# vitasoftAI/ImageRetrievalResearch

Measured on AMD Instinct MI355X. Metric: images/sec embed + queries/sec top-k@100k-gallery, EffNet-B3a 224^2, higher is better.
Workload: dtype bf16

## Files before the change

imageretrievalresearch_amd/csrc/gemm_bf16.hip:

```cpp
#include "ops.h"
#include "../../include/mi355_retrieval.h"

#include <stdlib.h>

namespace mi355 {

typedef __bf16 bf16x8 __attribute__((ext_vector_type(8)));
typedef float f32x4 __attribute__((ext_vector_type(4)));
typedef unsigned u32x4 __attribute__((ext_vector_type(4)));
typedef unsigned u32x2 __attribute__((ext_vector_type(2)));

__device__ __forceinline__ float lo_bf(unsigned u) { return __uint_as_float(u << 16); }
__device__ __forceinline__ float hi_bf(unsigned u) { return __uint_as_float(u & 0xffff0000u); }

__device__ __forceinline__ u32x4 gate_chunk(u32x4 v, const float* __restrict__ gp, int relu6) {
    const f32x4 g0 = *reinterpret_cast<const f32x4*>(gp);
    const f32x4 g1 = *reinterpret_cast<const f32x4*>(gp + 4);
    float f[8] = {lo_bf(v.x) * g0.x, hi_bf(v.x) * g0.y, lo_bf(v.y) * g0.z, hi_bf(v.y) * g0.w,
                  lo_bf(v.z) * g1.x, hi_bf(v.z) * g1.y, lo_bf(v.w) * g1.z, hi_bf(v.w) * g1.w};
    if (relu6) {
#pragma unroll
        for (int i = 0; i < 8; ++i) f[i] = fminf(fmaxf(f[i], 0.f), 6.f);
    }
    u32x4 o;
    o.x = pack2bf(f[0], f[1]); o.y = pack2bf(f[2], f[3]); o.z = pack2bf(f[4], f[5]); o.w = pack2bf(f[6], f[7]);
    return o;
}

__device__ __forceinline__ u32x4 gate_chunk_regs(u32x4 v, f32x4 g0, f32x4 g1, int relu6) {
    float f[8] = {lo_bf(v.x) * g0.x, hi_bf(v.x) * g0.y, lo_bf(v.y) * g0.z, hi_bf(v.y) * g0.w,
                  lo_bf(v.z) * g1.x, hi_bf(v.z) * g1.y, lo_bf(v.w) * g1.z, hi_bf(v.w) * g1.w};
    if (relu6) {
#pragma unroll
// ... 617 lines not shown
}

template <int NT, int KST>
__global__ __launch_bounds__(512) void k_proj_lds(const GemmArgs g) {
    constexpr int NW = 8;
    constexpr int KP = KST * 32;
    constexpr int WLD = KP + 8, ALD = KP + 8, CLD = NT * 16 + 8;
    extern __shared__ __attribute__((aligned(16))) unsigned char psm[];
    bf16_t* Wsh = reinterpret_cast<bf16_t*>(psm);
    float* sbias = reinterpret_cast<float*>(psm + (size_t)NT * 16 * WLD * 2);
    unsigned char* wbase = psm + (size_t)NT * 16 * WLD * 2 + NT * 16 * 4;
    constexpr int WS = 16 * ALD * 2 + 16 * CLD * 2 + KP * 4;
    const int tid = threadIdx.x, lane = tid & 63;
    const int wave = __builtin_amdgcn_readfirstlane(tid >> 6);
    bf16_t* As = reinterpret_cast<bf16_t*>(wbase + (size_t)wave * WS);
    bf16_t* Cs = As + 16 * ALD;
    float* Gs = reinterpret_cast<float*>(Cs + 16 * CLD);
    const int Npad = (g.N + 15) & ~15;
    for (int id = tid; id < NT * 16 * KST * 4; id += 512) {
        const int row = id / (KST * 4), c = id - row * (KST * 4);
        u32x4 v = {0u, 0u, 0u, 0u};
        if (row < Npad && c * 8 < g.ldw) v = *reinterpret_cast<const u32x4*>(g.W + (size_t)row * g.ldw + c * 8);
        *reinterpret_cast<u32x4*>(&Wsh[row * WLD + c * 8]) = v;
    }
    for (int n = tid; n < NT * 16; n += 512) sbias[n] = n < Npad ? g.bias[n] : 0.f;
    for (int id = lane; id < 16 * (ALD / 8); id += 64) *reinterpret_cast<u32x4*>(&As[id * 8]) = (u32x4){0u, 0u, 0u, 0u};
    __syncthreads();

    const int fr = lane & 15, fq = lane >> 4;
    const int kc = g.K >> 3;
    const int nchunk = 16 * kc;
    const int ntiles = (g.M + 15) >> 4;
    const int stride = gridDim.x * NW;
    int img = -1;
    u32x4 sv[KST];
    auto stage_load = [&](int tile) {
#pragma unroll
        for (int i = 0; i < KST; ++i) {
            const int id = min(lane + 64 * i, nchunk - 1);
            const int row = id / kc, c = id - row * kc;
            const int m = min(tile * 16 + row, g.M - 1);
            sv[i] = *reinterpret_cast<const u32x4*>(g.A + (size_t)m * g.lda + c * 8);
        }
        __builtin_amdgcn_sched_barrier(0);
    };
    int tile = blockIdx.x * NW + wave;
    if (tile < ntiles) stage_load(tile);
    for (; tile < ntiles; tile += stride) {
        if (g.gate) {
            const int im = (tile * 16) / g.rows_per_img;
            if (im != img) {
                img = im;
                for (int k4 = lane; k4 * 4 < g.K; k4 += 64)
                    *reinterpret_cast<f32x4*>(&Gs[k4 * 4]) = *reinterpret_cast<const f32x4*>(g.gate + (size_t)im * g.gate_ld + k4 * 4);
            }
        }
#pragma unroll
        for (int i = 0; i < KST; ++i) {
            const int id = lane + 64 * i;
            if (id < nchunk) {
                const int row = id / kc, c = id - row * kc;
                u32x4 v = sv[i];
                if (g.gate) v = gate_chunk(v, Gs + c * 8, g.a_relu6);
                else if (g.a_relu6) v = relu6_chunk(v);
                *reinterpret_cast<u32x4*>(&As[row * ALD + c * 8]) = v;
            }
        }
        if (tile + stride < ntiles) stage_load(tile + stride);
        f32x4 acc[NT];
#pragma unroll
        for (int ni = 0; ni < NT; ++ni) acc[ni] = (f32x4){0.f, 0.f, 0.f, 0.f};
#pragma unroll
        for (int ks = 0; ks < KST; ++ks) {
            const bf16x8 af = *reinterpret_cast<const bf16x8*>(&As[fr * ALD + ks * 32 + fq * 8]);
#pragma unroll
            for (int ni = 0; ni < NT; ++ni) {
                const bf16x8 wf = *reinterpret_cast<const bf16x8*>(&Wsh[(ni * 16 + fr) * WLD + ks * 32 + fq * 8]);
                acc[ni] = __builtin_amdgcn_mfma_f32_16x16x32_bf16(wf, af, acc[ni], 0, 0, 0);
            }
        }
        MI355_ACT_DISPATCH(g.act, {
_Pragma("unroll")
            for (int ni = 0; ni < NT; ++ni) {
                const f32x4 bb = *reinterpret_cast<const f32x4*>(&sbias[ni * 16 + fq * 4]);
                acc[ni].x = act_c<ACT>(acc[ni].x + bb.x); acc[ni].y = act_c<ACT>(acc[ni].y + bb.y);
                acc[ni].z = act_c<ACT>(acc[ni].z + bb.z); acc[ni].w = act_c<ACT>(acc[ni].w + bb.w);
            }
        })
        const int m = tile * 16 + fr;
#pragma unroll
        for (int ni = 0; ni < NT; ++ni) {
            const int n = ni * 16 + fq * 4;
            float v[4] = {acc[ni].x, acc[ni].y, acc[ni].z, acc[ni].w};
            if (g.res && m < g.M && n < g.N) {
                if (n + 3 < g.res_n) {
                    const u32x2 rr = *reinterpret_cast<const u32x2*>(g.res + (size_t)m * g.ldr + n);
                    v[0] += lo_bf(rr.x); v[1] += hi_bf(rr.x); v[2] += lo_bf(rr.y); v[3] += hi_bf(rr.y);
                } else {
#pragma unroll
                    for (int r = 0; r < 4; ++r)
                        if (n + r < g.res_n) v[r] += bf2f(g.res[(size_t)m * g.ldr + n + r]);
                }
            }
            u32x2 o;
            o.x = pack2bf(v[0], v[1]);
            o.y = pack2bf(v[2], v[3]);
            *reinterpret_cast<u32x2*>(&Cs[fr * CLD + n]) = o;
        }
        constexpr int CPR = NT * 2;
#pragma unroll
        for (int i = 0; i < (16 * CPR + 63) / 64; ++i) {
            const int id = lane + 64 * i;
            const int row = id / CPR, c = id - row * CPR;
            const int mm = tile * 16 + row;
            if (id < 16 * CPR && mm < g.M && c * 8 < g.N)
                *reinterpret_cast<u32x4*>((bf16_t*)g.out + (size_t)mm * g.ldo + c * 8) =
                    *reinterpret_cast<const u32x4*>(&Cs[row * CLD + c * 8]);
        }
    }
}

template <int NT, int KST>
static int launch_proj_cfg(const GemmArgs& a, hipStream_t st) {
    constexpr int KP = KST * 32;
    const size_t lds = (size_t)NT * 16 * (KP + 8) * 2 + (size_t)NT * 16 * 4 +
                       (size_t)8 * (16 * (KP + 8) * 2 + 16 * (NT * 16 + 8) * 2 + KP * 4);
    static bool attr_done[MI355_MAX_DEVICES] = {false};
    if (first_time_on_this_device(attr_done)) {
        MI355_CHECK_HIP(hipFuncSetAttribute((const void*)k_proj_lds<NT, KST>, hipFuncAttributeMaxDynamicSharedMemorySize,
                                            160 * 1024));
    }
    const int ntiles = cdiv(a.M, 16);
    int blocks = cdiv(ntiles, 8);
    if (blocks > 256 * 6) blocks = 256 * 6;
    hipLaunchKernelGGL((k_proj_lds<NT, KST>), dim3(blocks), dim3(512), lds, st, a);
    MI355_LAUNCH_CHECK();
    return OK;
}

static int try_launch_proj(const GemmArgs& a, hipStream_t st, int* nt_out) {
    if (a.out_f32 || a.M < (1 << 19) || a.N % 8 || a.ldo % 8 || a.N > 64 || a.K > 288 || a.lda != a.K) return -1;
    if (a.gate && (a.rows_per_img % 16 != 0 || a.gate_ld % 4 != 0)) return -1;
    const int kst = (a.K + 31) / 32, nt = (a.N + 15) / 16;
#define PROJ_CASE(NTV, KSTV) if (nt == NTV && kst == KSTV) { *nt_out = NTV; return launch_proj_cfg<NTV, KSTV>(a, st); }
    PROJ_CASE(2, 1); PROJ_CASE(2, 2); PROJ_CASE(2, 5); PROJ_CASE(2, 6); PROJ_CASE(3, 6); PROJ_CASE(3, 9); PROJ_CASE(2, 9);
    PROJ_CASE(4, 8); PROJ_CASE(3, 5);
#undef PROJ_CASE
    return -1;
}

static int try_launch_stream(const GemmArgs& a, hipStream_t st, int* nt_out) {
    if (a.out_f32 || a.M < 4096 || a.N % 8 || a.ldo % 8 || a.gate || a.a_relu6) return -1;
    const int kst = (a.K + 31) / 32;
    const int nt = (a.N + 15) / 16;
    *nt_out = nt;
    if (kst == 1 && nt == 9) return launch_stream_cfg<9, 1>(a, st);
    if (kst == 1 && nt == 12) return launch_stream_cfg<12, 1>(a, st);
    return -1;
}

constexpr int SK_KC = 256, SK_BM = 64, SK_BN = 64, SK_LD = SK_KC + 8;
constexpr size_t SK_MAX_BYTES = (size_t)64 << 20;

int gemm_splitk_chunks(long M, int rows_per_img, int N, int K) {
    if (M > 16384 || rows_per_img > 196 || K < 512 || N < 64 || N % 8 || gemm_splitk_bytes(M, N, K) > SK_MAX_BYTES) return 0;
    return (K + SK_KC - 1) / SK_KC;
}
size_t gemm_splitk_bytes(long M, int N, int K) {
    return (size_t)((K + SK_KC - 1) / SK_KC) * (size_t)M * (size_t)((N + 15) & ~15) * sizeof(float);
}

__global__ __launch_bounds__(256) void k_gemm_splitk(const GemmArgs g, float* __restrict__ ws) {
    extern __shared__ __attribute__((aligned(16))) bf16_t sksm[];
    bf16_t* As = sksm;
    bf16_t* Ws = sksm + SK_BM * SK_LD;
// ... 348 lines not shown
```

imageretrievalresearch_amd/csrc/sweep_mbconv.hip:

```cpp
#include "../../include/mi355_retrieval.h"
#include "ops.h"

namespace mi355 {

typedef __bf16 bf16x8 __attribute__((ext_vector_type(8)));
typedef float f32x4 __attribute__((ext_vector_type(4)));
typedef unsigned u32x4 __attribute__((ext_vector_type(4)));
typedef unsigned u32x2 __attribute__((ext_vector_type(2)));

__device__ __forceinline__ void sw_lds_barrier() {
    asm volatile("s_waitcnt lgkmcnt(0)" ::: "memory");
    __builtin_amdgcn_s_barrier();
    asm volatile("" ::: "memory");
}

typedef __bf16 sw_bf16x2 __attribute__((ext_vector_type(2)));
typedef float sw_f32x2 __attribute__((ext_vector_type(2)));
__device__ __forceinline__ u32x2 sw_pack4(const f32x4 v) {
    const sw_bf16x2 lo = __builtin_convertvector((sw_f32x2){v.x, v.y}, sw_bf16x2);
    const sw_bf16x2 hi = __builtin_convertvector((sw_f32x2){v.z, v.w}, sw_bf16x2);
    u32x2 o;
    o.x = *reinterpret_cast<const unsigned*>(&lo);
    o.y = *reinterpret_cast<const unsigned*>(&hi);
    return o;
}

template <int ACT>
__device__ __forceinline__ float sw_act(float x, int act_runtime) {
    if constexpr (ACT >= 0) return act_c<ACT>(x);
    else return apply_act(x, act_runtime);
}

template <int KS> struct SwTaps {
    static constexpr int NV = (KS / 2) * KS;
    static constexpr int NH = (KS + 1) / 2;
    static constexpr int NP = NV + NH;
    __host__ __device__ static constexpr bool vertical(int tp) { return tp < NV; }
    __host__ __device__ static constexpr int tap_a(int tp) {
        return tp < NV ? (tp / KS) * 2 * KS + tp % KS : (KS - 1) * KS + (tp - NV) * 2;
    }
    __host__ __device__ static constexpr int tap_b(int tp) {
        return tp < NV ? tap_a(tp) + KS : ((tp - NV) * 2 + 1 < KS ? tap_a(tp) + 1 : -1);
    }
};

template <int KS, int S, int WI, int TH>
struct SwGeom {
    static constexpr int PAD = KS / 2;
    static constexpr int HALO = KS - S;
    static constexpr int NEWR = TH * S;
    static constexpr int IH = NEWR + HALO;
    static constexpr int EW = WI + 2 * PAD;
    static constexpr int EWH = (EW + 1) / 2;
    static constexpr int RP = S == 1 ? EW : 2 * EWH;
    static constexpr int HOFF = S == 1 ? 1 : EWH;
    static constexpr int WO = (WI + 2 * PAD - KS) / S + 1;
    static constexpr int ELD = 24;
    static constexpr int EBUF = (IH + 1) * RP * ELD;
    static constexpr size_t lds_bytes(int nw, int ns = 1) { return (size_t)ns * 2 * EBUF * 2 + (size_t)nw * 16 * ns * 4; }
    __host__ __device__ static constexpr int epx(int r, int c) {
        return r * RP + (S == 1 ? c : (c & 1) * EWH + (c >> 1));
    }
};

template <int KS, int S, int WI, int TH, int NW, int KST, int OCC, bool PREF, int AE, int AD, int NS = 1>
__global__ __launch_bounds__(NW * 64, (NW * OCC + 3) / 4) void k_sweep_mbconv(const SweepArgs a) {
    using G = SwGeom<KS, S, WI, TH>;
    using TP = SwTaps<KS>;
    constexpr int NTHR = NW * 64;
    constexpr int PAD = G::PAD, HALO = G::HALO, NEWR = G::NEWR, RP = G::RP, ELD = G::ELD, WO = G::WO, NP = TP::NP;
    constexpr int NPX1 = NEWR * WI, NT1 = (NPX1 + 15) / 16, MW1 = (NT1 + NW - 1) / NW;
    constexpr int NPX2 = TH * WO, NT2 = (NPX2 + 15) / 16, MW2 = (NT2 + NW - 1) / NW;
    constexpr int EBUF = G::EBUF;
    extern __shared__ __attribute__((aligned(16))) unsigned char sw_smem[];
    bf16_t* Es = reinterpret_cast<bf16_t*>(sw_smem);
    float* red = reinterpret_cast<float*>(sw_smem + (size_t)NS * 2 * EBUF * 2);

    const int tid = threadIdx.x, lane = tid & 63;
    const int wave = __builtin_amdgcn_readfirstlane(tid >> 6);
    const int fr = lane & 15, fq = lane >> 4, fk = fq * 8;
    const int xcd = blockIdx.x & 7, seq = blockIdx.x >> 3;
    const int b = xcd + 8 * (seq / a.csplit), g = seq % a.csplit;
    if (b >= a.B) return;
    const int midp = (a.mid + 15) & ~15;
    const int nslab = (midp / 16 + NS - 1) / NS;
    const int nbands = (a.Ho + TH - 1) / TH;

    const bool stamping = a.stamps != nullptr;
    long long t_acc[10] = {0, 0, 0, 0, 0, 0, 0, 0, 0, 0};
    long long t_last = 0;
    if (stamping) t_last = (long long)__builtin_readcyclecounter();
    auto tick = [&](int i) {
        if (stamping) { const long long t = (long long)__builtin_readcyclecounter(); t_acc[i] += t - t_last; t_last = t; }
    };

    for (int id = tid; id < NS * 2 * EBUF / 8; id += NTHR) *reinterpret_cast<u32x4*>(&Es[id * 8]) = (u32x4){0u, 0u, 0u, 0u};

    int eoff[MW1];
#pragma unroll
    for (int i = 0; i < MW1; ++i) {
        const int p = min((wave + NW * i) * 16 + fr, NPX1 - 1);
        const int r = p / WI, x = p - r * WI;
        eoff[i] = G::epx(HALO + r, x + PAD) * ELD + fq * 4;
    }
    int rbase[MW2];
#pragma unroll
    for (int i = 0; i < MW2; ++i) {
        const int p = min((wave + NW * i) * 16 + fr, NPX2 - 1);
        const int oyl = p / WO, ox = p - oyl * WO;
        rbase[i] = (oyl * S * RP + ox) * ELD + (fq & 1) * 8;
    }
    const int vsel = (fq >> 1) ? RP * ELD : 0;
    const int hsel = (fq >> 1) ? G::HOFF * ELD : 0;
    sw_lds_barrier();
    tick(0);

    const bf16_t* xb = a.X + (size_t)b * a.H * WI * a.Cin;
    bf16_t* Db = a.D + (size_t)b * a.Ho * WO * a.mid;
    const int hw1 = a.H * WI - 1;
    const int kclamp = a.Cin - 8;

    u32x4 xa[MW1][KST];
    auto load_x = [&](int band) {
        const int pix0 = (band * NEWR - PAD + HALO) * WI;
#pragma unroll
        for (int i = 0; i < MW1; ++i) {
            const int pix = min(max(pix0 + (wave + NW * i) * 16 + fr, 0), hw1);
#pragma unroll
            for (int ks = 0; ks < KST; ++ks) {
                u32x4 t = {0u, 0u, 0u, 0u};
                if (!(a.debug_skip & 4)) t = *reinterpret_cast<const u32x4*>(xb + pix * a.Cin + min(ks * 32 + fk, kclamp));
                xa[i][ks] = t;
            }
        }
        __builtin_amdgcn_sched_barrier(0);
    };

    for (int si = g; si < nslab; si += a.csplit) {
        const int ch0 = ((si + b) % nslab) * (16 * NS);
        load_x(-1);
        if constexpr (HALO > NEWR) {
            constexpr int NZ16 = (HALO - NEWR) * RP * ELD / 8;
#pragma unroll
            for (int s = 0; s < NS; ++s)
                for (int id = tid; id < NZ16; id += NTHR)
                    *reinterpret_cast<u32x4*>(&Es[s * 2 * EBUF + NEWR * RP * ELD + id * 8]) = (u32x4){0u, 0u, 0u, 0u};
        }
        u32x4 wf[NS][KST];
        f32x4 bb[NS], bdr[NS];
        unsigned wd_raw[NS][(NP + 1) / 2];
#pragma unroll
        for (int s = 0; s < NS; ++s) {
            const int c0 = ch0 + 16 * s;
            const int n = min(c0 + fr, midp - 1);
#pragma unroll
            for (int ks = 0; ks < KST; ++ks) wf[s][ks] = *reinterpret_cast<const u32x4*>(a.We + (n * a.Kp + ks * 32 + fk));
            bb[s] = *reinterpret_cast<const f32x4*>(a.be + min(c0 + fq * 4, midp - 4));
            const int ch = min(c0 + fr, a.mid - 1);
#pragma unroll
            for (int tp = 0; tp < NP; ++tp) {
                const int ta = TP::tap_a(tp), tb = TP::tap_b(tp) < 0 ? TP::tap_a(tp) : TP::tap_b(tp);
                const unsigned v = a.Wd[((lane & 32) ? tb : ta) * a.mid + ch];
                if (tp & 1) wd_raw[s][tp >> 1] |= v << 16;
                else wd_raw[s][tp >> 1] = v;
            }
            bdr[s] = *reinterpret_cast<const f32x4*>(a.bd + min(c0 + fq * 4, a.mid - 4));
        }
        auto build_dwf = [&](int s, u32x4* dwf) {
            const bool mine = ((fq & 1) == (fr >> 3)) && (ch0 + 16 * s + fr < a.mid);
            const int q = (fr & 7) >> 1;
#pragma unroll
            for (int tp = 0; tp < NP; ++tp) {
                const bool has = mine && !((lane & 32) && TP::tap_b(tp) < 0);
                const unsigned v = has ? ((tp & 1) ? wd_raw[s][tp >> 1] >> 16 : wd_raw[s][tp >> 1] & 0xffffu) : 0u;
                const unsigned word = (fr & 1) ? (v << 16) : v;
                dwf[tp] = (u32x4){q == 0 ? word : 0u, q == 1 ? word : 0u, q == 2 ? word : 0u, q == 3 ? word : 0u};
            }
        };
        constexpr bool DWF_PER_SLAB = KS == 3;
        u32x4 dwf_s[NS][DWF_PER_SLAB ? NP : 1];
        float psum[NS][4];
#pragma unroll
        for (int s = 0; s < NS; ++s)
#pragma unroll
            for (int j = 0; j < 4; ++j) psum[s][j] = 0.f;
        asm volatile("s_waitcnt vmcnt(0)" ::: "memory");
#pragma unroll
        for (int s = 0; s < NS; ++s) {
#pragma unroll
            for (int ks = 0; ks < KST; ++ks) asm volatile("" : "+v"(wf[s][ks]));
            asm volatile("" : "+v"(bb[s]));
            asm volatile("" : "+v"(bdr[s]));
#pragma unroll
            for (int i = 0; i < (NP + 1) / 2; ++i) asm volatile("" : "+v"(wd_raw[s][i]));
        }
#pragma unroll
        for (int i = 0; i < MW1; ++i)
#pragma unroll
            for (int ks = 0; ks < KST; ++ks) asm volatile("" : "+v"(xa[i][ks]));
        if constexpr (DWF_PER_SLAB) {
#pragma unroll
            for (int s = 0; s < NS; ++s) build_dwf(s, dwf_s[s]);
        }
        tick(1);

        for (int band = -1; band < nbands; ++band) {
            bf16_t* Ec = Es + ((band + 1) & 1) * EBUF;
            {
                const int iyn0 = band * NEWR - PAD + HALO;
                const int plo = max(0, -iyn0) * WI, phi = max(0, min(NEWR, a.H - iyn0)) * WI;
                if (!PREF && band >= 0) load_x(band);
                tick(3);
                if (stamping) { asm volatile("s_waitcnt vmcnt(0)" ::: "memory"); tick(4); }
#pragma unroll
                for (int i = 0; i < MW1; ++i) {
                    const int t0 = (wave + NW * i) * 16;
                    if (t0 < NPX1 && (band >= 0 || t0 + 16 > (NEWR - HALO) * WI)) {
#pragma unroll
                        for (int s = 0; s < NS; ++s) {
                            u32x2 o = {0u, 0u};
                            if (t0 < phi && t0 + 16 > plo && !(a.debug_skip & 1)) {
                                f32x4 acc = bb[s];
#pragma unroll
                                for (int ks = 0; ks < KST; ++ks)
                                    acc = __builtin_amdgcn_mfma_f32_16x16x32_bf16(*reinterpret_cast<bf16x8*>(&wf[s][ks]),
                                                                                  *reinterpret_cast<bf16x8*>(&xa[i][ks]), acc, 0, 0, 0);
                                acc.x = sw_act<AE>(acc.x, a.act_e); acc.y = sw_act<AE>(acc.y, a.act_e);
                                acc.z = sw_act<AE>(acc.z, a.act_e); acc.w = sw_act<AE>(acc.w, a.act_e);
                                o = sw_pack4(acc);
                                if (t0 < plo || t0 + 16 > phi) {
                                    const bool in = t0 + fr >= plo && t0 + fr < phi;
                                    o.x = in ? o.x : 0u; o.y = in ? o.y : 0u;
                                }
                            }
                            if (t0 + fr < NPX1) *reinterpret_cast<u32x2*>(&Ec[s * 2 * EBUF + eoff[i]]) = o;
                        }
                    }
                }
                if (PREF && band + 1 < nbands) load_x(band + 1);
            }
            tick(5);
            sw_lds_barrier();
            tick(6);
            if (band + 1 < nbands) {
                bf16_t* En = Es + (band & 1) * EBUF;
                constexpr int NV16 = HALO * RP * ELD / 8;
#pragma unroll
                for (int s = 0; s < NS; ++s)
                    for (int id = tid; id < NV16; id += NTHR)
                        *reinterpret_cast<u32x4*>(&En[s * 2 * EBUF + id * 8]) = *reinterpret_cast<const u32x4*>(&Ec[s * 2 * EBUF + NEWR * RP * ELD + id * 8]);
            }
            tick(2);
#pragma unroll
            for (int s = 0; s < NS; ++s) {
            const int c0 = ch0 + 16 * s;
            if (band >= 0 && c0 < a.mid && !(a.debug_skip & 2)) {
                u32x4 dwf_b[DWF_PER_SLAB ? 1 : NP];
                if constexpr (!DWF_PER_SLAB) build_dwf(s, dwf_b);
                const u32x4* dwf = DWF_PER_SLAB ? dwf_s[s] : dwf_b;
                const int np2 = min(TH, a.Ho - band * TH) * WO;
                bf16_t* Dband = Db + band * NPX2 * a.mid + c0 + fq * 4;
                const bf16_t* Ecs = Ec + s * 2 * EBUF;
#pragma unroll
                for (int i = 0; i < MW2; ++i) {
                    const int t0 = (wave + NW * i) * 16;
                    if (t0 < np2) {
                        const bf16_t* ev = Ecs + rbase[i] + vsel;
                        const bf16_t* eh = Ecs + rbase[i] + hsel;
                        auto e_read = [&](int tp) -> bf16x8 {
                            const int ta = TP::tap_a(tp);
                            const int offs = G::epx(ta / KS, ta % KS) * ELD;
                            return *reinterpret_cast<const bf16x8*>((TP::vertical(tp) ? ev : eh) + offs);
                        };
                        constexpr int NB = KS == 5 ? 2 : NP, NG = (NP + NB - 1) / NB;
                        bf16x8 ef[2][NB];
#pragma unroll
                        for (int k = 0; k < NB; ++k)
                            if (k < NP) ef[0][k] = e_read(k);
                        f32x4 acc = bdr[s];
#pragma unroll
                        for (int gq = 0; gq < NG; ++gq) {
                            if (gq + 1 < NG) {
#pragma unroll
                                for (int k = 0; k < NB; ++k)
                                    if ((gq + 1) * NB + k < NP) ef[(gq + 1) & 1][k] = e_read((gq + 1) * NB + k);
                            }
                            __builtin_amdgcn_sched_barrier(0);
#pragma unroll
                            for (int k = 0; k < NB; ++k)
                                if (gq * NB + k < NP)
                                    acc = __builtin_amdgcn_mfma_f32_16x16x32_bf16(*reinterpret_cast<const bf16x8*>(&dwf[gq * NB + k]), ef[gq & 1][k], acc, 0, 0, 0);
                            __builtin_amdgcn_sched_barrier(0);
                        }
                        acc.x = sw_act<AD>(acc.x, a.act_d); acc.y = sw_act<AD>(acc.y, a.act_d);
                        acc.z = sw_act<AD>(acc.z, a.act_d); acc.w = sw_act<AD>(acc.w, a.act_d);
                        const int p = t0 + fr;
                        if (p < np2) {
                            psum[s][0] += acc.x; psum[s][1] += acc.y; psum[s][2] += acc.z; psum[s][3] += acc.w;
                            if (c0 + fq * 4 < a.mid) {
                                *reinterpret_cast<u32x2*>(Dband + p * a.mid) = sw_pack4(acc);
                            }
                        }
                    }
                }
            }
            }
            tick(7);
        }

        if (a.pool) {
#pragma unroll
            for (int s = 0; s < NS; ++s) {
#pragma unroll
                for (int o = 1; o < 16; o <<= 1) {
#pragma unroll
                    for (int j = 0; j < 4; ++j) psum[s][j] += __shfl_xor(psum[s][j], o, 64);
                }
                if (fr == 0) *reinterpret_cast<f32x4*>(&red[(wave * NS + s) * 16 + fq * 4]) = (f32x4){psum[s][0], psum[s][1], psum[s][2], psum[s][3]};
            }
            sw_lds_barrier();
            if (tid < 16 * NS) {
                const int s = tid >> 4, c = tid & 15;
                float sum = 0.f;
#pragma unroll
                for (int w = 0; w < NW; ++w) sum += red[(w * NS + s) * 16 + c];
                if (ch0 + tid < a.mid) a.pool[(size_t)b * a.mid + ch0 + tid] = sum;
            }
        }
        sw_lds_barrier();
        tick(9);
    }
    if (stamping && tid == 0) {
#pragma unroll
        for (int i = 0; i < 10; ++i) atomicAdd(reinterpret_cast<unsigned long long*>(a.stamps + (size_t)b * 16 + i), (unsigned long long)t_acc[i]);
    }
}

struct SwPlan { int cls; int wgs_per_cu; int nct; };

enum { SW_NONE = 0, SW_3_2_112, SW_3_1_56, SW_5_2_56, SW_5_1_28, SW_3_2_28, SW_3_2_56, SW_3_1_28 };
static_assert(SW_3_2_112 == MI355_SWEEP_CLASS_3_2_112 && SW_3_2_28 == MI355_SWEEP_CLASS_3_2_28 && SW_3_1_28 == MI355_SWEEP_CLASS_3_1_28, "sweep classes");

static int sw_class(int H, int W, int k, int stride) {
    if (k == 3 && stride == 2 && W == 112 && H == 112) return SW_3_2_112;
    if (k == 3 && stride == 1 && W == 56 && H == 56) return SW_3_1_56;
    if (k == 5 && stride == 2 && W == 56 && H == 56) return SW_5_2_56;
    if (k == 5 && stride == 1 && W == 28 && H == 28) return SW_5_1_28;
    if (k == 3 && stride == 2 && W == 28 && H == 28) return SW_3_2_28;
    if (k == 3 && stride == 2 && W == 56 && H == 56) return SW_3_2_56;
    if (k == 3 && stride == 1 && W == 28 && H == 28) return SW_3_1_28;
    return SW_NONE;
}

static bool sw_rex_instance(int cls, int kst) {
    return (cls == SW_3_2_56 && (kst == 2 || kst == 3)) || (cls == SW_3_1_28 && (kst == 3 || kst == 4)) || (cls == SW_3_2_28 && kst == 3);
}

bool sweep_mbconv_supported(int H, int W, int Cin, int mid, int k, int stride, int act_e, int act_d) {
    if (Cin % 8 || mid % 8 || Cin < 8) return false;
    const int cls = sw_class(H, W, k, stride), kst = (Cin + 31) / 32;
    if (cls == SW_NONE) return false;
    if (act_e == ACT_SILU && act_d == ACT_NONE && sw_rex_instance(cls, kst)) return true;
    return Cin <= 64 && cls <= SW_3_2_28;
}

template <int KS, int S, int WI, int TH, int NW, int KST, int OCC, bool PREF, int AE, int AD, int NS = 1>
static int launch_sw_act(SweepArgs a, int B, hipStream_t st, int* path, int cls, int variant) {
    using G = SwGeom<KS, S, WI, TH>;
    const size_t lds = G::lds_bytes(NW, NS);
    static_assert(G::lds_bytes(NW, NS) <= 160 * 1024, "sweep: the row windows do not fit the LDS");
    static bool attr_done[MI355_MAX_DEVICES] = {false};
    if (first_time_on_this_device(attr_done)) {
        MI355_CHECK_HIP(hipFuncSetAttribute((const void*)k_sweep_mbconv<KS, S, WI, TH, NW, KST, OCC, PREF, AE, AD, NS>,
                                            hipFuncAttributeMaxDynamicSharedMemorySize, 160 * 1024));
    }
    const int nslab = cdiv(cdiv(a.mid, 16), NS);
    const int slots = 256 * OCC;
    int c = WI >= 56 ? (WI == 112 ? 3 : 4) : 2;
    while (c < nslab && (nslab % c != 0 || (long)B * c < slots)) ++c;
    if (c > nslab) c = nslab;
    a.csplit = a.csplit_override > 0 ? std::min(a.csplit_override, nslab) : c;
    a.B = B;
    const unsigned grid = (unsigned)(8 * cdiv(B, 8) * a.csplit);
    hipLaunchKernelGGL((k_sweep_mbconv<KS, S, WI, TH, NW, KST, OCC, PREF, AE, AD, NS>), dim3(grid), dim3(NW * 64), lds, st, a);
    MI355_LAUNCH_CHECK();
    if (path) {
        const int inst = AE < 0 ? MI355_FRONT_ACT_RUNTIME : (AD == ACT_SILU ? MI355_FRONT_ACT_SILU_SILU : MI355_FRONT_ACT_SILU_NONE);
        *path = MI355_FRONT_PATH_SWEEP(KS, S, cls, KST, NS, variant, inst, a.csplit);
    }
    return OK;
}

template <int KS, int S, int WI, int TH, int NW, int KST, int OCC, bool PREF>
static int launch_sw(const SweepArgs& a, int B, hipStream_t st, int* path, int cls) {
    if (a.act_e == ACT_SILU && a.act_d == ACT_SILU) return launch_sw_act<KS, S, WI, TH, NW, KST, OCC, PREF, ACT_SILU, ACT_SILU>(a, B, st, path, cls, 0);
    if (a.act_e == ACT_SILU && a.act_d == ACT_NONE) return launch_sw_act<KS, S, WI, TH, NW, KST, OCC, PREF, ACT_SILU, ACT_NONE>(a, B, st, path, cls, 0);
    return launch_sw_act<KS, S, WI, TH, NW, KST, OCC, PREF, -1, -1>(a, B, st, path, cls, 0);
}

#define SW_V0(KS, S, WI, TH, NW, OCC, PREF) \
    return k2 ? launch_sw<KS, S, WI, TH, NW, 2, OCC, false>(a, B, st, path, cls) : launch_sw<KS, S, WI, TH, NW, 1, OCC, PREF>(a, B, st, path, cls)
#define SW_VT(KS, S, WI, TH, NW, KST, OCC, PREF) \
    return launch_sw_act<KS, S, WI, TH, NW, KST, OCC, PREF, ACT_SILU, ACT_SILU>(a, B, st, path, cls, v)

int launch_sweep_mbconv(const SweepArgs& a, int B, int k, int stride, hipStream_t st, int* path) {
    if (path) *path = 0;
    MI355_REQUIRE(sweep_mbconv_supported(a.H, a.W, a.Cin, a.mid, k, stride, a.act_e, a.act_d) && a.Kp % 32 == 0 && a.Kp >= 32 && a.Kp <= 128,
                  "sweep_mbconv: unsupported shape %dx%d k%d s%d Cin %d", a.H, a.W, k, stride, a.Cin);
    const bool k2 = a.Kp == 64;
    const bool silu = a.act_e == ACT_SILU && a.act_d == ACT_SILU;
    const int cls = sw_class(a.H, a.W, k, stride);
    if (a.act_e == ACT_SILU && a.act_d == ACT_NONE && (sw_rex_instance(cls, a.Kp / 32) || (cls == SW_3_1_56 && a.Kp == 64))) {
#define REX(KS, S, WI, TH, NW, KST, OCC, PREF, NS) return launch_sw_act<KS, S, WI, TH, NW, KST, OCC, PREF, ACT_SILU, ACT_NONE, NS>(a, B, st, path, cls, rv)
        const int kst = a.Kp / 32;
        int rv = 3;
        if (a.variant == 3) {
            if (cls == SW_3_1_56) REX(3, 1, 56, 8, 8, 2, 1, true, 1);
            if (cls == SW_3_2_56) { if (kst == 2) REX(3, 2, 56, 2, 7, 2, 1, true, 1); REX(3, 2, 56, 2, 7, 3, 2, false, 1); }
        }
        rv = 0;
        if (cls == SW_3_1_56) REX(3, 1, 56, 8, 8, 2, 1, true, 2);
        if (cls == SW_3_2_56) { if (kst == 2) REX(3, 2, 56, 2, 7, 2, 1, true, 2); REX(3, 2, 56, 2, 7, 3, 1, false, 2); }
        if (cls == SW_3_1_28) { if (kst == 3) REX(3, 1, 28, 4, 7, 3, 2, false, 1); REX(3, 1, 28, 4, 7, 4, 2, false, 1); }
        REX(3, 2, 28, 4, 7, 3, 2, false, 1);
#undef REX
    }
    MI355_REQUIRE(a.Kp <= 64 && cls <= SW_3_2_28, "sweep_mbconv: no instance for %dx%d k%d s%d Kp %d", a.H, a.W, k, stride, a.Kp);
    const int v = (silu && k2 == (cls == SW_5_1_28 || cls == SW_3_2_28)) ? a.variant : 0;
    switch (cls) {
        case SW_3_2_112:
            if (v == 1) SW_VT(3, 2, 112, 2, 7, 1, 2, true);
            if (v == 2) SW_VT(3, 2, 112, 2, 8, 1, 3, false);
            if (v == 3) SW_VT(3, 2, 112, 1, 7, 1, 2, true);
            if (v == 4) SW_VT(3, 2, 112, 1, 4, 1, 4, true);
            SW_V0(3, 2, 112, 2, 8, 2, true);
        case SW_3_1_56:
            if (v == 1) SW_VT(3, 1, 56, 8, 7, 1, 2, true);
            if (v == 2) SW_VT(3, 1, 56, 4, 8, 1, 2, true);
            if (v == 3) SW_VT(3, 1, 56, 2, 7, 1, 2, true);
            if (v == 4) SW_VT(3, 1, 56, 2, 7, 1, 3, true);
            SW_V0(3, 1, 56, 8, 8, 2, true);
        case SW_5_2_56:
            if (v == 1) SW_VT(5, 2, 56, 4, 7, 1, 2, true);
            if (v == 2) SW_VT(5, 2, 56, 2, 8, 1, 2, true);
            if (v == 3) SW_VT(5, 2, 56, 2, 7, 1, 2, false);
            if (v == 4) SW_VT(5, 2, 56, 1, 7, 1, 2, true);
            SW_V0(5, 2, 56, 2, 7, 2, true);
        case SW_5_1_28:
            if (v == 1) SW_VT(5, 1, 28, 4, 7, 2, 2, true);
            if (v == 2) SW_VT(5, 1, 28, 4, 8, 2, 2, false);
            if (v == 3) SW_VT(5, 1, 28, 2, 7, 2, 2, false);
            if (v == 4) SW_VT(5, 1, 28, 4, 4, 2, 4, false);
            SW_V0(5, 1, 28, 4, 7, 2, false);
        default:
            if (v == 1) SW_VT(3, 2, 28, 7, 7, 2, 2, false);
            if (v == 2) SW_VT(3, 2, 28, 4, 8, 2, 2, true);
            if (v == 3) SW_VT(3, 2, 28, 2, 7, 2, 2, true);
            if (v == 4) SW_VT(3, 2, 28, 4, 7, 2, 2, true);
            SW_V0(3, 2, 28, 4, 7, 2, false);
    }
}
#undef SW_V0
#undef SW_VT

}
```

Before: 60620.

## Prefetch residual and gate vectors into registers alongside A tile in proj kernel

The projection GEMM kernel now prefetches the residual tile and the per-image gate vector into registers in the same software-pipelined stage as the A tile, and stages the residual through LDS instead of issuing scattered per-lane global loads in the epilogue. Stores are made branch-free by clamping indices, and partial vmcnt waits are added so the next tile's loads overlap the current tile's output stores. The aim is to hide global-load latency for the residual and gate and to remove divergent epilogue loads. In exchange it uses more registers and adds redundant clamped loads and stores at boundaries. It also adds an alignment guard on the residual pointer.

```diff
diff --git a/imageretrievalresearch_amd/csrc/gemm_bf16.hip b/imageretrievalresearch_amd/csrc/gemm_bf16.hip
--- a/imageretrievalresearch_amd/csrc/gemm_bf16.hip
+++ b/imageretrievalresearch_amd/csrc/gemm_bf16.hip
@@ -1,4 +1,5 @@
 #include "ops.h"
+#include "proj_index.h"
 #include "../../include/mi355_retrieval.h"
 
 #include <stdlib.h>
@@ -682,38 +683,69 @@
     const int nchunk = 16 * kc;
     const int ntiles = (g.M + 15) >> 4;
     const int stride = gridDim.x * NW;
-    int img = -1;
-    u32x4 sv[KST];
+    constexpr int RR = (NT + 1) / 2;
+    constexpr int GR = (KST + 7) / 8;
+    constexpr int CPR = NT * 2;
+    constexpr int NST = (16 * CPR + 63) / 64;
+    const int rn = g.res ? min(g.res_n, g.N) : 0;
+    const int rc = g.res ? proj_res_chunks(g.res_n, g.N) : 1;
+    const bf16_t* rbase = g.res ? g.res : g.A;
+    const int rld = g.res ? g.ldr : 0;
+    const float* gbase = g.gate ? g.gate : reinterpret_cast<const float*>(g.A);
+    const int gld = g.gate ? g.gate_ld : 0, gk = g.gate ? g.K : 4, rpi = g.gate ? g.rows_per_img : 1 << 30;
+    u32x4 sv[KST], rv[RR];
+    f32x4 gv[GR];
     auto stage_load = [&](int tile) {
 #pragma unroll
-        for (int i = 0; i < KST; ++i) {
-            const int id = min(lane + 64 * i, nchunk - 1);
-            const int row = id / kc, c = id - row * kc;
-            const int m = min(tile * 16 + row, g.M - 1);
-            sv[i] = *reinterpret_cast<const u32x4*>(g.A + (size_t)m * g.lda + c * 8);
-        }
+        for (int i = 0; i < KST; ++i)
+            sv[i] = *reinterpret_cast<const u32x4*>(g.A + proj_chunk(tile, lane + 64 * i, kc, g.M, g.lda).off);
+#pragma unroll
+        for (int i = 0; i < RR; ++i)
+            rv[i] = *reinterpret_cast<const u32x4*>(rbase + proj_chunk(tile, lane + 64 * i, rc, g.M, rld).off);
+#pragma unroll
+        for (int i = 0; i < GR; ++i)
+            gv[i] = *reinterpret_cast<const f32x4*>(gbase + proj_gate_off(tile, lane + 64 * i, gk, rpi, gld));
         __builtin_amdgcn_sched_barrier(0);
     };
+    auto landed = [&]() {
+#pragma unroll
+        for (int i = 0; i < KST; ++i) asm volatile("" : "+v"(sv[i]));
+#pragma unroll
+        for (int i = 0; i < RR; ++i) asm volatile("" : "+v"(rv[i]));
+#pragma unroll
+        for (int i = 0; i < GR; ++i) asm volatile("" : "+v"(gv[i]));
+    };
     int tile = blockIdx.x * NW + wave;
-    if (tile < ntiles) stage_load(tile);
+    stage_load(min(tile, ntiles - 1));
+    asm volatile("s_waitcnt vmcnt(0)" ::: "memory");
+    landed();
     for (; tile < ntiles; tile += stride) {
         if (g.gate) {
-            const int im = (tile * 16) / g.rows_per_img;
-            if (im != img) {
-                img = im;
-                for (int k4 = lane; k4 * 4 < g.K; k4 += 64)
-                    *reinterpret_cast<f32x4*>(&Gs[k4 * 4]) = *reinterpret_cast<const f32x4*>(g.gate + (size_t)im * g.gate_ld + k4 * 4);
+#pragma unroll
+            for (int i = 0; i < GR; ++i) {
+                const int k4 = lane + 64 * i;
+                if (k4 * 4 < g.K) *reinterpret_cast<f32x4*>(&Gs[k4 * 4]) = gv[i];
             }
         }
 #pragma unroll
         for (int i = 0; i < KST; ++i) {
             const int id = lane + 64 * i;
             if (id < nchunk) {
-                const int row = id / kc, c = id - row * kc;
+                const ProjChunk p = proj_chunk(tile, id, kc, g.M, g.lda);
                 u32x4 v = sv[i];
-                if (g.gate) v = gate_chunk(v, Gs + c * 8, g.a_relu6);
+                if (g.gate) v = gate_chunk(v, Gs + p.c * 8, g.a_relu6);
                 else if (g.a_relu6) v = relu6_chunk(v);
-                *reinterpret_cast<u32x4*>(&As[row * ALD + c * 8]) = v;
+                *reinterpret_cast<u32x4*>(&As[p.row * ALD + p.c * 8]) = v;
+            }
+        }
+        if (g.res) {
+#pragma unroll
+            for (int i = 0; i < RR; ++i) {
+                const int id = lane + 64 * i;
+                if (id < 16 * rc) {
+                    const ProjChunk p = proj_chunk(tile, id, rc, g.M, rld);
+                    *reinterpret_cast<u32x4*>(&Cs[p.row * CLD + p.c * 8]) = rv[i];
+                }
             }
         }
         if (tile + stride < ntiles) stage_load(tile + stride);
@@ -737,36 +769,26 @@
                 acc[ni].z = act_c<ACT>(acc[ni].z + bb.z); acc[ni].w = act_c<ACT>(acc[ni].w + bb.w);
             }
         })
-        const int m = tile * 16 + fr;
 #pragma unroll
         for (int ni = 0; ni < NT; ++ni) {
             const int n = ni * 16 + fq * 4;
             float v[4] = {acc[ni].x, acc[ni].y, acc[ni].z, acc[ni].w};
-            if (g.res && m < g.M && n < g.N) {
-                if (n + 3 < g.res_n) {
-                    const u32x2 rr = *reinterpret_cast<const u32x2*>(g.res + (size_t)m * g.ldr + n);
-                    v[0] += lo_bf(rr.x); v[1] += hi_bf(rr.x); v[2] += lo_bf(rr.y); v[3] += hi_bf(rr.y);
-                } else {
-#pragma unroll
-                    for (int r = 0; r < 4; ++r)
-                        if (n + r < g.res_n) v[r] += bf2f(g.res[(size_t)m * g.ldr + n + r]);
-                }
-            }
+            const u32x2 rr = *reinterpret_cast<const u32x2*>(&Cs[fr * CLD + n]);
+            const float r[4] = {lo_bf(rr.x), hi_bf(rr.x), lo_bf(rr.y), hi_bf(rr.y)};
+#pragma unroll
+            for (int q = 0; q < 4; ++q) v[q] = n + q < rn ? v[q] + r[q] : v[q];
             u32x2 o;
             o.x = pack2bf(v[0], v[1]);
             o.y = pack2bf(v[2], v[3]);
             *reinterpret_cast<u32x2*>(&Cs[fr * CLD + n]) = o;
         }
-        constexpr int CPR = NT * 2;
-#pragma unroll
-        for (int i = 0; i < (16 * CPR + 63) / 64; ++i) {
-            const int id = lane + 64 * i;
-            const int row = id / CPR, c = id - row * CPR;
-            const int mm = tile * 16 + row;
-            if (id < 16 * CPR && mm < g.M && c * 8 < g.N)
-                *reinterpret_cast<u32x4*>((bf16_t*)g.out + (size_t)mm * g.ldo + c * 8) =
-                    *reinterpret_cast<const u32x4*>(&Cs[row * CLD + c * 8]);
-        }
+#pragma unroll
+        for (int i = 0; i < NST; ++i) {
+            const ProjChunk p = proj_store_chunk(tile, lane + 64 * i, CPR, g.M, g.N, g.ldo);
+            *reinterpret_cast<u32x4*>((bf16_t*)g.out + p.off) = *reinterpret_cast<const u32x4*>(&Cs[p.row * CLD + p.c * 8]);
+        }
+        asm volatile("s_waitcnt vmcnt(%0)" ::"n"(NST) : "memory");
+        landed();
     }
 }
 
@@ -791,6 +813,7 @@
 static int try_launch_proj(const GemmArgs& a, hipStream_t st, int* nt_out) {
     if (a.out_f32 || a.M < (1 << 19) || a.N % 8 || a.ldo % 8 || a.N > 64 || a.K > 288 || a.lda != a.K) return -1;
     if (a.gate && (a.rows_per_img % 16 != 0 || a.gate_ld % 4 != 0)) return -1;
+    if (a.res && (a.ldr % 8 != 0 || a.ldr < a.res_n || (reinterpret_cast<uintptr_t>(a.res) & 15) != 0)) return -1;
     const int kst = (a.K + 31) / 32, nt = (a.N + 15) / 16;
 #define PROJ_CASE(NTV, KSTV) if (nt == NTV && kst == KSTV) { *nt_out = NTV; return launch_proj_cfg<NTV, KSTV>(a, st); }
     PROJ_CASE(2, 1); PROJ_CASE(2, 2); PROJ_CASE(2, 5); PROJ_CASE(2, 6); PROJ_CASE(3, 6); PROJ_CASE(3, 9); PROJ_CASE(2, 9);
diff --git a/imageretrievalresearch_amd/csrc/proj_index.h b/imageretrievalresearch_amd/csrc/proj_index.h
--- /dev/null
+++ b/imageretrievalresearch_amd/csrc/proj_index.h
@@ -0,0 +1,47 @@
+#pragma once
+
+#if defined(__HIPCC__) || defined(__CUDACC__)
+#define MI355_HD __host__ __device__
+#else
+#define MI355_HD
+#endif
+
+namespace mi355 {
+
+struct ProjChunk {
+    int row, c;
+    long off;
+};
+
+MI355_HD inline ProjChunk proj_chunk(int tile, int id, int cpr, int M, int ld) {
+    const int last = 16 * cpr - 1;
+    id = id < last ? id : last;
+    ProjChunk p;
+    p.row = id / cpr;
+    p.c = id - p.row * cpr;
+    const int m = tile * 16 + p.row;
+    p.off = (long)(m < M - 1 ? m : M - 1) * ld + p.c * 8;
+    return p;
+}
+
+MI355_HD inline ProjChunk proj_store_chunk(int tile, int id, int cpr, int M, int N, int ldo) {
+    const int last = 16 * cpr - 1;
+    id = id < last ? id : last;
+    const int lastrow = M - 1 - tile * 16 < 15 ? M - 1 - tile * 16 : 15;
+    ProjChunk p;
+    p.row = id / cpr;
+    p.c = id - p.row * cpr;
+    if (p.row > lastrow) p.row = lastrow;
+    if (p.c * 8 >= N) p.c = 0;
+    p.off = (long)(tile * 16 + p.row) * ldo + p.c * 8;
+    return p;
+}
+
+MI355_HD inline long proj_gate_off(int tile, int id, int K, int rows_per_img, int gate_ld) {
+    const int last = (K >> 2) - 1;
+    return (long)((tile * 16) / rows_per_img) * gate_ld + (id < last ? id : last) * 4;
+}
+
+MI355_HD inline int proj_res_chunks(int res_n, int N) { return ((res_n < N ? res_n : N) + 7) >> 3; }
+
+}
```

Result: no change. 60910, median of 3 (+0.5%).

## Stage per-slab weights into LDS via async DMA and prefetch across slabs

Applied to the files above, without the earlier changes.

The last wave of each workgroup now copies the next channel slab's expand weights, biases and depthwise weights into a double-buffered LDS region using global_load_lds DMA while the current slab computes. The first band of input for the next slab is prefetched at the tail of the previous slab, and the E double-buffer parity carries over between slabs. The pool reduction is deferred to one pass at kernel end, which removes a barrier per slab. In exchange LDS use grows with the slab count, which may lower occupancy or trip the new size check, and the hand-written vmcnt accounting is fragile.

```diff
diff --git a/imageretrievalresearch_amd/csrc/sweep_mbconv.hip b/imageretrievalresearch_amd/csrc/sweep_mbconv.hip
--- a/imageretrievalresearch_amd/csrc/sweep_mbconv.hip
+++ b/imageretrievalresearch_amd/csrc/sweep_mbconv.hip
@@ -1,5 +1,6 @@
 #include "../../include/mi355_retrieval.h"
 #include "ops.h"
+#include <type_traits>
 
 namespace mi355 {
 
@@ -12,6 +13,26 @@
     asm volatile("s_waitcnt lgkmcnt(0)" ::: "memory");
     __builtin_amdgcn_s_barrier();
     asm volatile("" ::: "memory");
+}
+
+__device__ __forceinline__ void sw_dma16(const void* gsrc, unsigned lds_dst) {
+    unsigned keep;
+    asm volatile("s_mov_b32 %0, m0\n\ts_mov_b32 m0, %2\n\ts_nop 0\n\tglobal_load_lds_dwordx4 %1, off\n\ts_mov_b32 m0, %0"
+                 : "=&s"(keep) : "v"(gsrc), "s"(lds_dst) : "memory");
+}
+__device__ __forceinline__ void sw_dma4(const void* gsrc, unsigned lds_dst) {
+    unsigned keep;
+    asm volatile("s_mov_b32 %0, m0\n\ts_mov_b32 m0, %2\n\ts_nop 0\n\tglobal_load_lds_dword %1, off\n\ts_mov_b32 m0, %0"
+                 : "=&s"(keep) : "v"(gsrc), "s"(lds_dst) : "memory");
+}
+
+template <int N>
+__device__ __forceinline__ void sw_wait_vm_leaving(int n) {
+    if constexpr (N == 0) asm volatile("s_waitcnt vmcnt(0)" ::: "memory");
+    else {
+        if (n >= N) asm volatile("s_waitcnt vmcnt(%0)" ::"n"(N) : "memory");
+        else sw_wait_vm_leaving<N - 1>(n);
+    }
 }
 
 typedef __bf16 sw_bf16x2 __attribute__((ext_vector_type(2)));
@@ -57,7 +78,11 @@
     static constexpr int WO = (WI + 2 * PAD - KS) / S + 1;
     static constexpr int ELD = 24;
     static constexpr int EBUF = (IH + 1) * RP * ELD;
-    static constexpr size_t lds_bytes(int nw, int ns = 1) { return (size_t)ns * 2 * EBUF * 2 + (size_t)nw * 16 * ns * 4; }
+    static constexpr int NWD = (KS * KS * 8 + 63) / 64;
+    static constexpr int cst_bytes(int kst) { return kst * 1024 + 128 + NWD * 256; }
+    static constexpr size_t lds_bytes(int nw, int ns, int kst, int nwalk) {
+        return (size_t)2 * ns * cst_bytes(kst) + (size_t)ns * 2 * EBUF * 2 + (size_t)nwalk * nw * 16 * ns * 4;
+    }
     __host__ __device__ static constexpr int epx(int r, int c) {
         return r * RP + (S == 1 ? c : (c & 1) * EWH + (c >> 1));
     }
@@ -73,12 +98,14 @@
     constexpr int NPX2 = TH * WO, NT2 = (NPX2 + 15) / 16, MW2 = (NT2 + NW - 1) / NW;
     constexpr int EBUF = G::EBUF;
     extern __shared__ __attribute__((aligned(16))) unsigned char sw_smem[];
-    bf16_t* Es = reinterpret_cast<bf16_t*>(sw_smem);
-    float* red = reinterpret_cast<float*>(sw_smem + (size_t)NS * 2 * EBUF * 2);
+    constexpr int NWD = G::NWD, CST = G::cst_bytes(KST);
+    const unsigned char* cst = sw_smem;
+    bf16_t* Es = reinterpret_cast<bf16_t*>(sw_smem + 2 * NS * CST);
+    float* red = reinterpret_cast<float*>(sw_smem + 2 * NS * CST + (size_t)NS * 2 * EBUF * 2);
 
     const int tid = threadIdx.x, lane = tid & 63;
     const int wave = __builtin_amdgcn_readfirstlane(tid >> 6);
-    const int fr = lane & 15, fq = lane >> 4, fk = fq * 8;
+    const int fr = lane & 15, fq = lane >> 4;
     const int xcd = blockIdx.x & 7, seq = blockIdx.x >> 3;
     const int b = xcd + 8 * (seq / a.csplit), g = seq % a.csplit;
     if (b >= a.B) return;
@@ -94,6 +121,61 @@
         if (stamping) { const long long t = (long long)__builtin_readcyclecounter(); t_acc[i] += t - t_last; t_last = t; }
     };
 
+    const bf16_t* xb = a.X + (size_t)b * a.H * WI * a.Cin;
+    bf16_t* Db = a.D + (size_t)b * a.Ho * WO * a.mid;
+    const int hw1 = a.H * WI - 1;
+    const int kclamp = a.Cin - 8;
+
+    u32x4 xa[MW1][KST];
+    auto load_x_of = [&](int band, auto first) {
+        constexpr bool FIRST = decltype(first)::value;
+        const int pix0 = (band * NEWR - PAD + HALO) * WI;
+        int l = lane;
+        if constexpr (FIRST) asm volatile("" : "+v"(l));
+        const int lr = l & 15, lk = (l >> 4) * 8;
+#pragma unroll
+        for (int i = 0; i < MW1; ++i) {
+            const int pix = min(max(pix0 + (wave + NW * i) * 16 + lr, 0), hw1);
+#pragma unroll
+            for (int ks = 0; ks < KST; ++ks) {
+                u32x4 t = {0u, 0u, 0u, 0u};
+                if (!(a.debug_skip & 4)) t = *reinterpret_cast<const u32x4*>(xb + pix * a.Cin + min(ks * 32 + lk, kclamp));
+                xa[i][ks] = t;
+            }
+        }
+        __builtin_amdgcn_sched_barrier(0);
+    };
+
+    auto ch0_of = [&](int si) { return ((si + b) % nslab) * (16 * NS); };
+    const unsigned cst_lds = (unsigned)(size_t)(__attribute__((address_space(3))) unsigned char*)sw_smem;
+    auto stage_consts = [&](int ch0, int set) {
+        int l = lane;
+        asm volatile("" : "+v"(l));
+        const int lr = l & 15, lk = (l >> 4) * 8;
+#pragma unroll
+        for (int s = 0; s < NS; ++s) {
+            const int c0 = ch0 + 16 * s;
+            const unsigned dst = cst_lds + (set * NS + s) * CST;
+            const int n = min(c0 + lr, midp - 1);
+#pragma unroll
+            for (int ks = 0; ks < KST; ++ks) sw_dma16(a.We + (n * a.Kp + ks * 32 + lk), dst + ks * 1024);
+            if (l < 8) {
+                const int q = l & 3;
+                const float* src = l < 4 ? a.be + min(c0 + q * 4, midp - 4) : a.bd + min(c0 + q * 4, a.mid - 4);
+                sw_dma16(src, dst + KST * 1024);
+            }
+#pragma unroll
+            for (int j = 0; j < NWD; ++j) {
+                const int t = min(j * 8 + (l >> 3), KS * KS - 1);
+                sw_dma4(a.Wd + (t * a.mid + min(c0 + 2 * (l & 7), a.mid - 2)), dst + KST * 1024 + 128 + j * 256);
+            }
+        }
+    };
+    u32x4 wf[NS][KST];
+    f32x4 bb[NS];
+    if (wave == NW - 1) stage_consts(ch0_of(g), 0);
+    if (PREF) load_x_of(-1, std::true_type{});
+
     for (int id = tid; id < NS * 2 * EBUF / 8; id += NTHR) *reinterpret_cast<u32x4*>(&Es[id * 8]) = (u32x4){0u, 0u, 0u, 0u};
 
     int eoff[MW1];
@@ -112,60 +194,51 @@
     }
     const int vsel = (fq >> 1) ? RP * ELD : 0;
     const int hsel = (fq >> 1) ? G::HOFF * ELD : 0;
+    if (wave == NW - 1) asm volatile("s_waitcnt vmcnt(0)" ::: "memory");
     sw_lds_barrier();
     tick(0);
 
-    const bf16_t* xb = a.X + (size_t)b * a.H * WI * a.Cin;
-    bf16_t* Db = a.D + (size_t)b * a.Ho * WO * a.mid;
-    const int hw1 = a.H * WI - 1;
-    const int kclamp = a.Cin - 8;
-
-    u32x4 xa[MW1][KST];
-    auto load_x = [&](int band) {
-        const int pix0 = (band * NEWR - PAD + HALO) * WI;
-#pragma unroll
-        for (int i = 0; i < MW1; ++i) {
-            const int pix = min(max(pix0 + (wave + NW * i) * 16 + fr, 0), hw1);
-#pragma unroll
-            for (int ks = 0; ks < KST; ++ks) {
-                u32x4 t = {0u, 0u, 0u, 0u};
-                if (!(a.debug_skip & 4)) t = *reinterpret_cast<const u32x4*>(xb + pix * a.Cin + min(ks * 32 + fk, kclamp));
-                xa[i][ks] = t;
-            }
-        }
-        __builtin_amdgcn_sched_barrier(0);
-    };
-
-    for (int si = g; si < nslab; si += a.csplit) {
-        const int ch0 = ((si + b) % nslab) * (16 * NS);
-        load_x(-1);
+    int pb = 0;
+    int kslab = 0;
+    int nst = 0;
+    for (int si = g; si < nslab; si += a.csplit, ++kslab) {
+        const int ch0 = ch0_of(si);
+        const bool has_next = si + a.csplit < nslab;
         if constexpr (HALO > NEWR) {
             constexpr int NZ16 = (HALO - NEWR) * RP * ELD / 8;
 #pragma unroll
             for (int s = 0; s < NS; ++s)
                 for (int id = tid; id < NZ16; id += NTHR)
-                    *reinterpret_cast<u32x4*>(&Es[s * 2 * EBUF + NEWR * RP * ELD + id * 8]) = (u32x4){0u, 0u, 0u, 0u};
-        }
-        u32x4 wf[NS][KST];
-        f32x4 bb[NS], bdr[NS];
+                    *reinterpret_cast<u32x4*>(&Es[(s * 2 + pb) * EBUF + NEWR * RP * ELD + id * 8]) = (u32x4){0u, 0u, 0u, 0u};
+        }
+        if (!PREF) load_x_of(-1, std::true_type{});
+        f32x4 bdr[NS];
         unsigned wd_raw[NS][(NP + 1) / 2];
+        int l = lane;
+        asm volatile("" : "+v"(l));
 #pragma unroll
         for (int s = 0; s < NS; ++s) {
-            const int c0 = ch0 + 16 * s;
-            const int n = min(c0 + fr, midp - 1);
-#pragma unroll
-            for (int ks = 0; ks < KST; ++ks) wf[s][ks] = *reinterpret_cast<const u32x4*>(a.We + (n * a.Kp + ks * 32 + fk));
-            bb[s] = *reinterpret_cast<const f32x4*>(a.be + min(c0 + fq * 4, midp - 4));
-            const int ch = min(c0 + fr, a.mid - 1);
+            const unsigned char* cs = cst + ((kslab & 1) * NS + s) * CST;
+#pragma unroll
+            for (int ks = 0; ks < KST; ++ks) wf[s][ks] = *reinterpret_cast<const u32x4*>(cs + ks * 1024 + l * 16);
+            bb[s] = *reinterpret_cast<const f32x4*>(cs + KST * 1024 + (l >> 4) * 16);
+            bdr[s] = *reinterpret_cast<const f32x4*>(cs + KST * 1024 + 64 + (l >> 4) * 16);
+            const unsigned short* wds = reinterpret_cast<const unsigned short*>(cs + KST * 1024 + 128) + (l & 15);
 #pragma unroll
             for (int tp = 0; tp < NP; ++tp) {
                 const int ta = TP::tap_a(tp), tb = TP::tap_b(tp) < 0 ? TP::tap_a(tp) : TP::tap_b(tp);
-                const unsigned v = a.Wd[((lane & 32) ? tb : ta) * a.mid + ch];
+                const unsigned v = wds[((l & 32) ? tb : ta) * 16];
                 if (tp & 1) wd_raw[s][tp >> 1] |= v << 16;
                 else wd_raw[s][tp >> 1] = v;
             }
-            bdr[s] = *reinterpret_cast<const f32x4*>(a.bd + min(c0 + fq * 4, a.mid - 4));
-        }
+        }
+        if (PREF) sw_wait_vm_leaving<MW2 * NS>(nst);
+        else asm volatile("s_waitcnt vmcnt(0)" ::: "memory");
+#pragma unroll
+        for (int i = 0; i < MW1; ++i)
+#pragma unroll
+            for (int ks = 0; ks < KST; ++ks) asm volatile("" : "+v"(xa[i][ks]));
+        if (has_next && wave == NW - 1) stage_consts(ch0_of(si + a.csplit), (kslab + 1) & 1);
         auto build_dwf = [&](int s, u32x4* dwf) {
             const bool mine = ((fq & 1) == (fr >> 3)) && (ch0 + 16 * s + fr < a.mid);
             const int q = (fr & 7) >> 1;
@@ -184,20 +257,6 @@
         for (int s = 0; s < NS; ++s)
 #pragma unroll
             for (int j = 0; j < 4; ++j) psum[s][j] = 0.f;
-        asm volatile("s_waitcnt vmcnt(0)" ::: "memory");
-#pragma unroll
-        for (int s = 0; s < NS; ++s) {
-#pragma unroll
-            for (int ks = 0; ks < KST; ++ks) asm volatile("" : "+v"(wf[s][ks]));
-            asm volatile("" : "+v"(bb[s]));
-            asm volatile("" : "+v"(bdr[s]));
-#pragma unroll
-            for (int i = 0; i < (NP + 1) / 2; ++i) asm volatile("" : "+v"(wd_raw[s][i]));
-        }
-#pragma unroll
-        for (int i = 0; i < MW1; ++i)
-#pragma unroll
-            for (int ks = 0; ks < KST; ++ks) asm volatile("" : "+v"(xa[i][ks]));
         if constexpr (DWF_PER_SLAB) {
 #pragma unroll
             for (int s = 0; s < NS; ++s) build_dwf(s, dwf_s[s]);
@@ -205,11 +264,11 @@
         tick(1);
 
         for (int band = -1; band < nbands; ++band) {
-            bf16_t* Ec = Es + ((band + 1) & 1) * EBUF;
+            bf16_t* Ec = Es + ((band + 1 + pb) & 1) * EBUF;
             {
                 const int iyn0 = band * NEWR - PAD + HALO;
                 const int plo = max(0, -iyn0) * WI, phi = max(0, min(NEWR, a.H - iyn0)) * WI;
-                if (!PREF && band >= 0) load_x(band);
+                if (!PREF && band >= 0) load_x_of(band, std::false_type{});
                 tick(3);
                 if (stamping) { asm volatile("s_waitcnt vmcnt(0)" ::: "memory"); tick(4); }
 #pragma unroll
@@ -237,13 +296,18 @@
                         }
                     }
                 }
-                if (PREF && band + 1 < nbands) load_x(band + 1);
+                const bool last = band + 1 >= nbands;
+                if (last && has_next && wave == NW - 1) asm volatile("s_waitcnt vmcnt(0)" ::: "memory");
+                if (PREF && (!last || has_next)) {
+                    load_x_of(last ? -1 : band + 1, std::false_type{});
+                    if (last) nst = 0;
+                }
             }
             tick(5);
             sw_lds_barrier();
             tick(6);
             if (band + 1 < nbands) {
-                bf16_t* En = Es + (band & 1) * EBUF;
+                bf16_t* En = Es + ((band + pb) & 1) * EBUF;
                 constexpr int NV16 = HALO * RP * ELD / 8;
 #pragma unroll
                 for (int s = 0; s < NS; ++s)
@@ -301,6 +365,7 @@
                                 *reinterpret_cast<u32x2*>(Dband + p * a.mid) = sw_pack4(acc);
                             }
                         }
+                        ++nst;
                     }
                 }
             }
@@ -316,18 +381,22 @@
 #pragma unroll
                     for (int j = 0; j < 4; ++j) psum[s][j] += __shfl_xor(psum[s][j], o, 64);
                 }
-                if (fr == 0) *reinterpret_cast<f32x4*>(&red[(wave * NS + s) * 16 + fq * 4]) = (f32x4){psum[s][0], psum[s][1], psum[s][2], psum[s][3]};
-            }
-            sw_lds_barrier();
-            if (tid < 16 * NS) {
-                const int s = tid >> 4, c = tid & 15;
-                float sum = 0.f;
-#pragma unroll
-                for (int w = 0; w < NW; ++w) sum += red[(w * NS + s) * 16 + c];
-                if (ch0 + tid < a.mid) a.pool[(size_t)b * a.mid + ch0 + tid] = sum;
-            }
-        }
+                if (fr == 0) *reinterpret_cast<f32x4*>(&red[((kslab * NW + wave) * NS + s) * 16 + fq * 4]) = (f32x4){psum[s][0], psum[s][1], psum[s][2], psum[s][3]};
+            }
+        }
+        pb = (pb + nbands + 1) & 1;
+        tick(9);
+    }
+    if (a.pool && g < nslab) {
         sw_lds_barrier();
+        for (int id = tid; id < kslab * 16 * NS; id += NTHR) {
+            const int k = id / (16 * NS), t = id - k * (16 * NS);
+            const int ch = ch0_of(g + k * a.csplit) + t;
+            float sum = 0.f;
+#pragma unroll
+            for (int w = 0; w < NW; ++w) sum += red[(k * NW + w) * (16 * NS) + t];
+            if (ch < a.mid) a.pool[(size_t)b * a.mid + ch] = sum;
+        }
         tick(9);
     }
     if (stamping && tid == 0) {
@@ -367,8 +436,7 @@
 template <int KS, int S, int WI, int TH, int NW, int KST, int OCC, bool PREF, int AE, int AD, int NS = 1>
 static int launch_sw_act(SweepArgs a, int B, hipStream_t st, int* path, int cls, int variant) {
     using G = SwGeom<KS, S, WI, TH>;
-    const size_t lds = G::lds_bytes(NW, NS);
-    static_assert(G::lds_bytes(NW, NS) <= 160 * 1024, "sweep: the row windows do not fit the LDS");
+    static_assert(G::lds_bytes(NW, NS, KST, 1) <= 160 * 1024, "sweep: the row windows do not fit the LDS");
     static bool attr_done[MI355_MAX_DEVICES] = {false};
     if (first_time_on_this_device(attr_done)) {
         MI355_CHECK_HIP(hipFuncSetAttribute((const void*)k_sweep_mbconv<KS, S, WI, TH, NW, KST, OCC, PREF, AE, AD, NS>,
@@ -381,6 +449,8 @@
     if (c > nslab) c = nslab;
     a.csplit = a.csplit_override > 0 ? std::min(a.csplit_override, nslab) : c;
     a.B = B;
+    const size_t lds = G::lds_bytes(NW, NS, KST, cdiv(nslab, a.csplit));
+    MI355_REQUIRE(lds <= 160 * 1024, "sweep_mbconv: %d slabs per workgroup do not fit the LDS (%zu bytes)", cdiv(nslab, a.csplit), lds);
     const unsigned grid = (unsigned)(8 * cdiv(B, 8) * a.csplit);
     hipLaunchKernelGGL((k_sweep_mbconv<KS, S, WI, TH, NW, KST, OCC, PREF, AE, AD, NS>), dim3(grid), dim3(NW * 64), lds, st, a);
     MI355_LAUNCH_CHECK();
@@ -398,8 +468,8 @@
     return launch_sw_act<KS, S, WI, TH, NW, KST, OCC, PREF, -1, -1>(a, B, st, path, cls, 0);
 }
 
-#define SW_V0(KS, S, WI, TH, NW, OCC, PREF) \
-    return k2 ? launch_sw<KS, S, WI, TH, NW, 2, OCC, false>(a, B, st, path, cls) : launch_sw<KS, S, WI, TH, NW, 1, OCC, PREF>(a, B, st, path, cls)
+#define SW_V0(KS, S, WI, TH, NW, OCC, PREF, PREF2) \
+    return k2 ? launch_sw<KS, S, WI, TH, NW, 2, OCC, PREF2>(a, B, st, path, cls) : launch_sw<KS, S, WI, TH, NW, 1, OCC, PREF>(a, B, st, path, cls)
 #define SW_VT(KS, S, WI, TH, NW, KST, OCC, PREF) \
     return launch_sw_act<KS, S, WI, TH, NW, KST, OCC, PREF, ACT_SILU, ACT_SILU>(a, B, st, path, cls, v)
 
@@ -433,31 +503,31 @@
             if (v == 2) SW_VT(3, 2, 112, 2, 8, 1, 3, false);
             if (v == 3) SW_VT(3, 2, 112, 1, 7, 1, 2, true);
             if (v == 4) SW_VT(3, 2, 112, 1, 4, 1, 4, true);
-            SW_V0(3, 2, 112, 2, 8, 2, true);
+            SW_V0(3, 2, 112, 2, 8, 2, true, false);
         case SW_3_1_56:
             if (v == 1) SW_VT(3, 1, 56, 8, 7, 1, 2, true);
             if (v == 2) SW_VT(3, 1, 56, 4, 8, 1, 2, true);
             if (v == 3) SW_VT(3, 1, 56, 2, 7, 1, 2, true);
             if (v == 4) SW_VT(3, 1, 56, 2, 7, 1, 3, true);
-            SW_V0(3, 1, 56, 8, 8, 2, true);
+            SW_V0(3, 1, 56, 8, 8, 2, true, false);
         case SW_5_2_56:
             if (v == 1) SW_VT(5, 2, 56, 4, 7, 1, 2, true);
             if (v == 2) SW_VT(5, 2, 56, 2, 8, 1, 2, true);
             if (v == 3) SW_VT(5, 2, 56, 2, 7, 1, 2, false);
             if (v == 4) SW_VT(5, 2, 56, 1, 7, 1, 2, true);
-            SW_V0(5, 2, 56, 2, 7, 2, true);
+            SW_V0(5, 2, 56, 2, 7, 2, true, false);
         case SW_5_1_28:
             if (v == 1) SW_VT(5, 1, 28, 4, 7, 2, 2, true);
             if (v == 2) SW_VT(5, 1, 28, 4, 8, 2, 2, false);
             if (v == 3) SW_VT(5, 1, 28, 2, 7, 2, 2, false);
             if (v == 4) SW_VT(5, 1, 28, 4, 4, 2, 4, false);
-            SW_V0(5, 1, 28, 4, 7, 2, false);
+            SW_V0(5, 1, 28, 4, 7, 2, false, false);
         default:
             if (v == 1) SW_VT(3, 2, 28, 7, 7, 2, 2, false);
             if (v == 2) SW_VT(3, 2, 28, 4, 8, 2, 2, true);
             if (v == 3) SW_VT(3, 2, 28, 2, 7, 2, 2, true);
             if (v == 4) SW_VT(3, 2, 28, 4, 7, 2, 2, true);
-            SW_V0(3, 2, 28, 4, 7, 2, false);
+            SW_V0(3, 2, 28, 4, 7, 2, false, true);
     }
 }
 #undef SW_V0
```

Result: faster. 60250 before, 61650 after, median of 6 (+2.3%).
